# Gaeric/bevy-hikari

Measured on AMD Instinct MI355X. Metric: Mrays/sec + ms/frame @1080p 1spp; cornell & city scenes, 1/2/4/8 GPU, higher is better.
Workload: dtype f32

## Files before the change

### bevy-hikari_amd/csrc/hk_kernels.hip

```cpp
#include <stdlib.h>
#include <mutex>
#include <type_traits>

#include "hk_device.h"
#include "hk_launch.h"

namespace hk {

#ifdef HK_LANE_STATS
__device__ unsigned long long hk_lane_stats_dev[2 * LANE_SLOTS];
#endif
bool lane_stats_take(unsigned long long out[2 * LANE_SLOTS], hipStream_t st)
{
#ifdef HK_LANE_STATS
    unsigned long long zero[2 * LANE_SLOTS] = {};
    if (hipStreamSynchronize(st) != hipSuccess) return false;
    if (hipMemcpyFromSymbol(out, HIP_SYMBOL(hk_lane_stats_dev), sizeof(zero)) != hipSuccess) return false;
    return hipMemcpyToSymbol(HIP_SYMBOL(hk_lane_stats_dev), zero, sizeof(zero)) == hipSuccess;
#else
    (void)st;
    for (int k = 0; k < 2 * LANE_SLOTS; ++k) out[k] = 0;
    return false;
#endif
}
// ... 2320 lines not shown
    const bool window = A.F.upscale_ratio == 1.0f && A.F.s[0] == A.F.S[0] && A.F.s[1] == A.F.S[1];
    auto launch = [&](auto EL, auto VIEW) {
        if (window) hipLaunchKernelGGL((k_spatial<EL, VIEW>), g, dim3(256), 0, st, A, C);
        else hipLaunchKernelGGL((k_spatial_nowin<EL, VIEW>), g, dim3(256), 0, st, A, C);
    };
    if (emissive_lit) launch(std::true_type{}, std::false_type{});
    else dispatch([&](auto VIEW) { launch(std::false_type{}, VIEW); }, C.view != nullptr);
}
void launch_demod(const FrameArgs& A, const DenoiseArgs& D, hipStream_t st)
{
    dim3 g = tiles(A.F, A.F.s[0], A.F.s_rows);
    dispatch([&](auto C3) { hipLaunchKernelGGL((k_demod3<C3 ? 3 : 2>), g, dim3(256), 0, st, A, D); }, D.channels == 3);
}
template <int C, int LEVEL>
static void launch_level(const FrameArgs& A, const DenoiseArgs& D, hipStream_t st)
{
    const dim3 g = level_tiles<LEVEL>(launch_cols(A.F, A.F.s[0]), launch_rows(A.F, A.F.s_rows));
    hipLaunchKernelGGL((k_denoise3<C, LEVEL>), g, dim3(256), 0, st, A, D);
}
void launch_denoise(const FrameArgs& A, const DenoiseArgs& D, int level, hipStream_t st)
{
    dispatch(
        [&](auto C3) {
            constexpr int C = C3 ? 3 : 2;
            switch (level) {
            case 0: launch_level<C, 0>(A, D, st); break;
            case 1: launch_level<C, 1>(A, D, st); break;
            case 2: launch_level<C, 2>(A, D, st); break;
            default: launch_level<C, 3>(A, D, st); break;
            }
        },
        D.channels == 3);
}
void launch_tone(const FrameArgs& A, const ToneArgs& T, hipStream_t st)
{
    const Frame& F = A.F;
    const int32_t ly0 = F.win_rows > 0 ? F.win_row0 : 0, rows = launch_rows(F, F.s_rows);
    const int32_t x0 = F.win_cols > 0 ? F.win_col0 : 0, cols = (int32_t)launch_cols(F, F.s[0]);
    if (F.s[0] % (uint32_t)TONE_RUN == 0u && x0 % TONE_RUN == 0 && cols % TONE_RUN == 0 && rows > 0 && cols > 0) {
        const uint32_t runs = (uint32_t)cols / (uint32_t)TONE_RUN, n = runs * (uint32_t)rows;
        hipLaunchKernelGGL(k_tone_run, dim3((n + 255u) / 256u), dim3(256), 0, st, A, T, ly0, x0, runs, n);
    } else {
        hipLaunchKernelGGL(k_tone, tiles(A.F, A.F.s[0], A.F.s_rows), dim3(256), 0, st, A, T);
    }
}
__global__ __launch_bounds__(256) void k_accumulate(const uint2* tone, float4* acc, uint32_t n, int reset)
{
    uint32_t i = blockIdx.x * 256u + threadIdx.x;
    if (i >= n) return;
    f4 t = load_rgba16f(tone, (int32_t)i);
    float4 a = reset ? make_float4(0, 0, 0, 0) : acc[i];
    acc[i] = make_float4(a.x + t.x, a.y + t.y, a.z + t.z, a.w + t.w);
}
__global__ __launch_bounds__(256) void k_resolve(const float4* acc, uint32_t n, float count, uint2* out)
{
    uint32_t i = blockIdx.x * 256u + threadIdx.x;
    if (i >= n) return;
    float4 a = acc[i];
    store_rgba16f(out, (int32_t)i, mk4(a.x / count, a.y / count, a.z / count, a.w / count));
}
void launch_accumulate(const uint2* tone, float4* acc, uint32_t n, int reset, hipStream_t st)
{
    if (n) hipLaunchKernelGGL(k_accumulate, dim3((n + 255u) / 256u), dim3(256), 0, st, tone, acc, n, reset);
}
void launch_resolve(const float4* acc, uint32_t n, float count, uint2* out, hipStream_t st)
{
    if (n) hipLaunchKernelGGL(k_resolve, dim3((n + 255u) / 256u), dim3(256), 0, st, acc, n, count, out);
}

__global__ __launch_bounds__(256) void k_fill_blas_leaves(hk_node* nodes, uint32_t n, const uint32_t* prim_offset,
                                                          const hk_primitive* prims)
{
// ... 276 lines not shown
```

### bevy-hikari_amd/csrc/hk_launch.h

```cpp
#pragma once

#include <hip/hip_runtime.h>
#include <stdint.h>

#include "hk_device.h"
#include "../../include/hk_post.h"
#include "../../include/hk_fsr.h"
#include "../../include/hk_overlay.h"

namespace hk {

struct LaunchOpts {
    int lds_scene = 1;
    int gbuffer_stack_full = 0;
    int gbuffer_deep = 0;
    double gbuffer_lds_max_px = 6e5;
    double direct_w4_min_px = 4e5;
    int fused_w4 = 1;
    int persistent_indirect = 0;
    int compact_emitter = 0;
    int compact_shadow = 0;
};

struct FrameArgs {
// ... 184 lines not shown
    hk_pp_out out;
    hk_fsr_easu_con easu;
    float rcas;
};
void launch_fsr_easu(const FsrArgs& A, bool tiled, hipStream_t st);
void launch_fsr_rcas(const FsrArgs& A, hipStream_t st);

struct OverlayArgs {
    hk_pp_tex in, albedo;
    uint8_t* data;
    uint32_t pitch;
    hk_overlay_view view;
    uint32_t col0, cols;
};
void launch_overlay(const OverlayArgs& A, bool run, hipStream_t st);

bool lane_stats_take(unsigned long long out[2 * LANE_SLOTS], hipStream_t st);
void launch_gbuffer(const FrameArgs& A, const ViewArgs& V, uint2* albedo, uint32_t stack_need, hipStream_t st);
void launch_direct_fused(const FrameArgs& A, const ChannelArgs& C0, const ChannelArgs& C1, hipStream_t st,
                         const TileKeep& keep = TILE_KEEP_ALL);
void launch_albedo(const FrameArgs& A, uint2* albedo, hipStream_t st);
void launch_direct(const FrameArgs& A, const ChannelArgs& C, bool emissive_lit, hipStream_t st,
                   const TileKeep& keep = TILE_KEEP_ALL);
void launch_indirect(const FrameArgs& A, const ChannelArgs& C, bool multi, hipStream_t st, const TileKeep& keep = TILE_KEEP_ALL);
uint32_t indirect_stash_bytes();
void launch_indirect_wavefront(const FrameArgs& A, const ChannelArgs& C, const WfArgs& W, hipStream_t st);
void launch_spatial(const FrameArgs& A, const ChannelArgs& C, bool emissive_lit, hipStream_t st);
bool light_lds_direct(const FrameArgs& A);
void launch_light_merged(const FrameArgs& A, const ChannelArgs& C0, const ChannelArgs& C1, const ChannelArgs& C2,
                         hipStream_t st, const TileKeep& keep_direct = TILE_KEEP_ALL,
                         const TileKeep& keep_indirect = TILE_KEEP_ALL);
void launch_demod(const FrameArgs& A, const DenoiseArgs& D, hipStream_t st);
void launch_denoise(const FrameArgs& A, const DenoiseArgs& D, int level, hipStream_t st);
void launch_tone(const FrameArgs& A, const ToneArgs& T, hipStream_t st);
void launch_collapse_leaves(hk_node* nodes, uint32_t n, const uint32_t* node_base, const uint32_t* node_count,
                            uint32_t* scratch, hipStream_t st);
void launch_fill_leaves(hk_node* blas, uint32_t n_blas, const uint32_t* prim_offset, const hk_primitive* prims,
                        hk_node* tlas, uint32_t n_tlas, const hk_instance* inst, uint32_t n_inst, hipStream_t st);
void launch_build_wide(const hk_node* flat, uint32_t n, const uint32_t* node_base, const uint32_t* node_count,
                       float4* wide, hipStream_t st);
void launch_accumulate(const uint2* tone, float4* acc, uint32_t n, int reset, hipStream_t st);
void launch_resolve(const float4* acc, uint32_t n, float count, uint2* out, hipStream_t st);
void launch_div_check(float d, float r, uint32_t lo, uint32_t hi, unsigned long long* bad, hipStream_t st);
void launch_rcp_check(uint32_t lo, uint32_t hi, unsigned long long* bad, hipStream_t st);
void launch_count_check(const uint32_t* values, uint32_t n, unsigned long long* sum, hipStream_t st);
void launch_f16(const float* in, uint32_t n, uint16_t* out, hipStream_t st);
bool launch_math(int fn, const uint32_t* a, const uint32_t* b, const float* rb, uint32_t n, uint32_t* out0,
                 uint32_t* out1, hipStream_t st);
void launch_texture_check(const Scene& sc, uint32_t id, const float* uv, uint32_t n, float* out, hipStream_t st);
void launch_trace(const Scene& sc, const float* rays, const float* max_d, const float* early_d, const uint32_t* excl,
                  uint32_t n, uint32_t* hits, unsigned long long* top, hipStream_t st);

}
```

### bevy-hikari_amd/csrc/hk_runtime.hip

```cpp
#include <hip/hip_runtime.h>

#include <algorithm>
#include <array>
#include <cmath>
#include <cstdio>
#include <cstring>
#include <map>
#include <set>
#include <string>
#include <vector>

#include "../../include/hikari_amd.h"
#include "../../include/hikari_scene.h"
#include "hk_launch.h"

using namespace hk;

namespace {
constexpr int32_t BAND_HALO = 40;
constexpr size_t COUNTER_SPAN = (size_t)COUNTER_SHARDS * COUNTER_STRIDE;
constexpr size_t COUNTER_BYTES = 3 * COUNTER_SPAN * sizeof(unsigned long long);
constexpr size_t PERSIST_BYTES = (size_t)PERSIST_KINDS * PERSIST_LINES * PERSIST_LINE * sizeof(unsigned long long);

struct TimedLaunch {
// ... 203 lines not shown
        return PxRect{std::min(x0, o.x0), std::min(y0, o.y0), std::max(x1, o.x1), std::max(y1, o.y1)};
    }
};
struct MaskHistory {
    static constexpr int BITS = 5;
    PxRect cover[BITS];
    bool known[BITS] = {};
    void reset()
    {
        for (bool& k : known) k = false;
    }
    bool launch(uint32_t need, const PxRect& now, PxRect& keep)
    {
        bool ok = true;
        keep = now;
        for (int b = 0; b < BITS; ++b) {
            if (!(need >> b & 1u)) continue;
            if (!known[b]) ok = false;
            else keep = keep.join(cover[b]);
        }
        for (int b = 0; b < BITS; ++b) {
            if (need >> b & 1u) {
                cover[b] = now;
                known[b] = true;
            } else if (b == 4) {
                known[b] = false;
            } else if (known[b]) {
                cover[b] = cover[b].join(now);
            }
        }
        return ok;
    }
};
}

struct hk_ctx {
    int device = 0;
    hipStream_t stream = nullptr;
    std::string error;
    double opt[OPT_COUNT];
    bool on(Opt o) const { return opt[o] != 0.0; }

    void* buf[9] = {};
    uint32_t count[9] = {};
    hk_node* walk_nodes[2] = {nullptr, nullptr};
    uint32_t* collapse_scratch = nullptr;
    float4* blas_wide = nullptr;
    float4* tlas_wide = nullptr;
    uint32_t gb_stack_need = 0;
    bool heavy = false;
    int dn_calls = 0;
    uint32_t gb_blas_depth = 0;
    void* dyn_scratch = nullptr;
    size_t dyn_bytes = 0;
    struct MeshSlice {
        hk_mesh_index index;
        uint32_t vertex_need;
        uint32_t depth;
        uint32_t used = 0;
    };
    std::vector<MeshSlice> meshes;
    size_t cap[9] = {};
    size_t collapse_cap = 0;
    std::vector<float> emissive;
    uint32_t* blas_aux = nullptr;
    size_t aux_stride = 0;
// ... 13 lines not shown
    float* tex_lut = nullptr;
    uint32_t n_textures = 0;

    uint32_t S[2] = {0, 0}, s[2] = {0, 0};
    float ratio = 1.0f;
    int32_t S_row0 = 0, S_rows = 0, s_row0 = 0, s_rows = 0;
    int32_t core_row0 = 0, core_rows = 0;
    int32_t halo = BAND_HALO;
    int32_t stripe_n = 0, stripe_k = 0;
    bool albedo_fresh = false;
    bool sized = false;

    GSlot g, g_prev;
    FrameSchedule sch;
    uint32_t head = 0;
    float* variance[3] = {}, *variance_alt[3] = {};
    uint2* render[3] = {}, *render_alt[3] = {};
    uint4* reservoirs[HK_RESERVOIR_BUFFERS] = {};
    uint32_t res_n = 0;
    uint8_t* bgmask[2] = {};
    bool bg_valid[2] = {false, false};
    int32_t win_out = -1, win_emi = -1, win_ind = -1;
    int32_t core_col0 = 0, core_cols = 0;
    int32_t bg_key[2][2] = {};
    uint8_t* gbmask = nullptr;
    uint4* sp_view = nullptr;
    bool gb_valid = false;
    int32_t gb_key[2] = {};
    double scene_box[6] = {};
    bool scene_box_valid = false;
    PxRect grect[2] = {PxRect::all(), PxRect::all()};
    MaskHistory gb_hist, bg_hist[2];
    uint32_t tiles_skipped[3] = {};
    uint4* dn_rgb[4] = {};
    uint2* dn_bi[4] = {};
    float* internal_variance[3] = {};
    float4* dn_nd = nullptr;
    float4* dn_center = nullptr;
    float* dn_den2 = nullptr;
    int last_denoised_channels = 3;
    uint2* denoised[3] = {};
    uint2* tone_buf[2] = {};
    uint2* upscale = nullptr;
    uint2* taa_buf[2] = {};
    uint32_t upscale_wh[2] = {0, 0}, taa_wh[2] = {0, 0};
    uint2* fsr_buf[2] = {};
    float fsr_sharpness = 0.0f;
    uint8_t* present_buf = nullptr;
    uint32_t present_wh[2] = {0, 0}, present_format = 0;
    float4* accum = nullptr;
    uint2* accum_out = nullptr;
    uint32_t accum_n = 0;
    unsigned long long* counters = nullptr;
    unsigned long long* persist = nullptr;
    bool wavefront = false;
    uint32_t* wf_queue1 = nullptr;
    uint32_t* wf_keys = nullptr;
    uint32_t* wf_queue2 = nullptr;
    uint4* wf_hit = nullptr;
    float* wf_hit_t = nullptr;
    uint32_t* wf_ctl = nullptr;
    uint32_t wf_seg_cap = 0;

    struct GbSig {
        float view[3 + 16 + 16 + 16 + 2];
        int32_t win[2];
// ... 105 lines not shown
    for (auto& r : c->reservoirs) add(r, 's', 4);
    for (auto& m : c->bgmask) add(m, 's', 1, false);
    add(c->gbmask, 'S', 1, false);
    add(c->sp_view, 's', VIEW_PLANES);
    for (int i = 0; i < 4; ++i) {
        add(c->dn_rgb[i], 's');
        add(c->dn_bi[i], 's');
    }
    add(c->dn_nd, 's');
    add(c->dn_center, 's');
    add(c->dn_den2, 's');
    for (auto& b : c->tone_buf) add(b, 's');
    add(c->upscale, 0);
    for (auto& b : c->taa_buf) add(b, 0);
    for (auto& b : c->fsr_buf) add(b, 0);
    add(c->present_buf, 0);
    add(c->accum, 0);
    add(c->accum_out, 0);
    add(c->wf_queue1, 0);
    add(c->wf_keys, 0);
    add(c->wf_queue2, 0);
    add(c->wf_hit, 0);
    add(c->wf_hit_t, 0);
    add(c->wf_ctl, 0);
    return t;
}

void free_targets(hk_ctx* c)
{
    for (const Target& t : targets(c)) release(*t.ptr);
    c->bg_valid[0] = c->bg_valid[1] = c->gb_valid = false;
    c->grect[0] = c->grect[1] = PxRect::all();
    c->tiles_skipped[0] = c->tiles_skipped[1] = c->tiles_skipped[2] = 0;
    c->upscale_wh[0] = c->upscale_wh[1] = c->taa_wh[0] = c->taa_wh[1] = 0;
    c->present_wh[0] = c->present_wh[1] = 0;
    c->accum_n = 0;
    c->sch.reset();
    c->sized = false;
}

int ensure_wavefront(hk_ctx* c)
{
    if (c->wf_ctl) return HK_OK;
    const size_t n = (size_t)c->s[0] * (size_t)c->s_rows;
    const size_t tiles = (size_t)((c->s[0] + 15u) / 16u) * (size_t)(((uint32_t)c->s_rows + 15u) / 16u);
    c->wf_seg_cap = (uint32_t)(256u * ((tiles + WF_SEGS - 1u) / WF_SEGS));
    HK_HIP(c, hipMalloc(&c->wf_queue1, (size_t)WF_SEGS * c->wf_seg_cap * 4));
    HK_HIP(c, hipMalloc(&c->wf_keys, (size_t)WF_SEGS * c->wf_seg_cap * 4));
    HK_HIP(c, hipMalloc(&c->wf_queue2, n * 4));
    HK_HIP(c, hipMalloc(&c->wf_hit, n * sizeof(uint4)));
    HK_HIP(c, hipMalloc(&c->wf_hit_t, n * 4));
    HK_HIP(c, hipMalloc(&c->wf_ctl, (size_t)wf_ctl_words(WF_MAX_BINS) * 4));
    return HK_OK;
}

hipEvent_t take_event(hk_ctx* c)
{
    if (!c->event_pool.empty()) {
        hipEvent_t e = c->event_pool.back();
        c->event_pool.pop_back();
        return e;
    }
    hipEvent_t e = nullptr;
    (void)hipEventCreate(&e);
    return e;
}
// ... 272 lines not shown
    if (!G.grows) return HK_OK;
    commit_growth(c, G);
    if (!G.fill) return HK_OK;
    const size_t w = c->s[0];
    for (int b = 0; b < HK_RESERVOIR_BUFFERS; ++b)
        for (int side = 0; side < 2; ++side) {
            const int32_t r0 = G.rows[b][side][0], r1 = G.rows[b][side][1];
            if (r1 <= r0) continue;
            for (uint32_t plane = 0; plane < 4; ++plane)
                HK_HIP(c, hipMemsetAsync(c->reservoirs[b] + (size_t)plane * c->res_n + (size_t)r0 * w, 0,
                                         (size_t)(r1 - r0) * w * sizeof(uint4), s));
        }
    c->bg_valid[0] = c->bg_valid[1] = false;
    return HK_OK;
}


uint64_t gbuffer_primary_rays(const FrameArgs& A)
{
    const Frame& F = A.F;
    const int32_t w0 = F.win_rows > 0 ? F.win_row0 : 0, w1 = w0 + launch_rows(F, F.S_rows);
    if (F.stripe_n >= 2) return (uint64_t)F.S[0] * (uint64_t)(w1 - w0);
    const int32_t lo = std::max(F.S_row0 + w0, F.count_Sy0), hi = std::min(F.S_row0 + w1, F.count_Sy1);
    const int32_t c0 = F.win_cols > 0 ? F.win_col0 : 0, c1 = c0 + (int32_t)launch_cols(F, F.S[0]);
    const int32_t x0 = std::max(c0, F.count_x0), x1 = std::min(c1, F.count_x1);
    return hi > lo && x1 > x0 ? (uint64_t)(x1 - x0) * (uint64_t)(hi - lo) : 0u;
}

TileKeep tile_keep(const FrameArgs& A, uint32_t width, int32_t row0, int32_t rows, const PxRect& keep, uint32_t* skipped)
{
    const Frame& F = A.F;
    *skipped = 0;
    if (F.stripe_n >= 2) return TILE_KEEP_ALL;
    const int64_t ox = F.win_cols > 0 ? F.win_col0 : 0, oy = (int64_t)row0 + (F.win_rows > 0 ? F.win_row0 : 0);
    const int64_t gx = (launch_cols(F, width) + 15u) / 16u, gy = ((uint32_t)launch_rows(F, rows) + 15u) / 16u;
    auto lo = [](int64_t p, int64_t o, int64_t g) { return std::clamp<int64_t>(p - o, 0, 16 * g) / 16; };
    auto hi = [](int64_t p, int64_t o, int64_t g) { return (std::clamp<int64_t>(p - o, 0, 16 * g) + 15) / 16; };
    TileKeep K{(uint32_t)lo(keep.x0, ox, gx), (uint32_t)lo(keep.y0, oy, gy), (uint32_t)hi(keep.x1, ox, gx),
               (uint32_t)hi(keep.y1, oy, gy)};
    if (keep.empty() || K.x1 <= K.x0 || K.y1 <= K.y0) K = TileKeep{0u, 0u, 0u, 0u};
    *skipped = (uint32_t)(gx * gy) - (K.x1 - K.x0) * (K.y1 - K.y0);
    return *skipped ? K : TILE_KEEP_ALL;
}
uint64_t gbuffer_skipped_rays(const FrameArgs& A, const TileKeep& K)
{
    const Frame& F = A.F;
    const uint64_t all = gbuffer_primary_rays(A);
    if (K.x1 <= K.x0 || K.y1 <= K.y0) return all;
    const int32_t w0 = F.win_rows > 0 ? F.win_row0 : 0, w1 = w0 + launch_rows(F, F.S_rows);
    const int32_t c0 = F.win_cols > 0 ? F.win_col0 : 0, c1 = c0 + (int32_t)launch_cols(F, F.S[0]);
    const int32_t ky0 = std::min<int64_t>(w0 + 16 * (int64_t)K.y0, w1), ky1 = std::min<int64_t>(w0 + 16 * (int64_t)K.y1, w1);
    const int32_t kx0 = std::min<int64_t>(c0 + 16 * (int64_t)K.x0, c1), kx1 = std::min<int64_t>(c0 + 16 * (int64_t)K.x1, c1);
    const int32_t lo = std::max(F.S_row0 + ky0, F.count_Sy0), hi = std::min(F.S_row0 + ky1, F.count_Sy1);
    const int32_t x0 = std::max(kx0, F.count_x0), x1 = std::min(kx1, F.count_x1);
    const uint64_t kept = hi > lo && x1 > x0 ? (uint64_t)(x1 - x0) * (uint64_t)(hi - lo) : 0u;
    return all - kept;
}

int check_ready(hk_ctx* c, bool need_scene)
{
    if (!c) return HK_ERR_INVALID;
    if (!c->sized) return fail(c, HK_ERR_STATE, "hk_resize has not been called");
    if (need_scene && !c->has_scene) return fail(c, HK_ERR_STATE, "no scene uploaded (hk_scene_upload)");
    if (need_scene && !c->has_noise) return fail(c, HK_ERR_STATE, "no blue noise uploaded (hk_set_noise)");
    return HK_OK;
}

}

extern "C" {

int hk_abi_version(void) { return HK_ABI_VERSION; }

// ... 1411 lines not shown
{
    if (!c || !capacity) return HK_ERR_INVALID;
    if (!c->has_scene) return HK_ERR_STATE;
    for (int i = 0; i < 9; ++i) capacity[i] = (uint32_t)c->cap[i];
    return HK_OK;
}

int hk_scene_shared_transform(const hk_ctx* c, int32_t* shared)
{
    if (!c || !shared) return HK_ERR_INVALID;
    if (!c->has_scene) return HK_ERR_STATE;
    *shared = c->shared_transform ? 1 : 0;
    return HK_OK;
}

int hk_tile_skip_info(const hk_ctx* c, uint32_t skipped[3], int32_t bound[4], int32_t* bounded)
{
    if (!c) return HK_ERR_INVALID;
    if (!c->sized) return HK_ERR_STATE;
    if (skipped)
        for (int k = 0; k < 3; ++k) skipped[k] = c->tiles_skipped[k];
    const PxRect& r = c->grect[c->sch.gslot];
    const bool none = r.x1 == INT32_MAX;
    if (bound) {
        bound[0] = none ? 0 : r.x0;
        bound[1] = none ? 0 : r.y0;
        bound[2] = none ? (int32_t)c->S[0] : r.x1;
        bound[3] = none ? (int32_t)c->S[1] : r.y1;
    }
    if (bounded) *bounded = none ? 0 : 1;
    return HK_OK;
}

int hk_instance_set_counts(const hk_scene_desc* d, const hk_instance_desc* set, uint32_t count,
                           const hk_material* materials, uint32_t counts[9])
{
    if (!d || !set || !counts || !scene_desc_ok(d)) return HK_ERR_INVALID;
    const uint32_t before[9] = {d->vertices.count,  d->primitives.count,     d->asset_nodes.count,
                                d->alias_table.count, d->instances.count,    d->instance_nodes.count,
                                d->materials.count, d->emissive_nodes.count, d->emissives.count};
    std::vector<hk_ctx::MeshSlice> known;
    std::set<std::array<uint32_t, 4>> seen;
    const hk_instance* inst = (const hk_instance*)d->instances.data;
    for (uint32_t k = 0; k < d->instances.count; ++k) {
        const hk_mesh_index& m = inst[k].mesh;
        if ((size_t)m.node[0] + m.node[1] > d->asset_nodes.count) return HK_ERR_INVALID;
        if (seen.insert({m.vertex, m.primitive, m.node[0], m.node[1]}).second) known.push_back(host_mesh_slice(d, m));
    }
    std::vector<float> emissive(4 * (size_t)d->materials.count);
    const hk_material* mats = materials ? materials : (const hk_material*)d->materials.data;
    for (uint32_t k = 0; k < d->materials.count; ++k) std::memcpy(&emissive[4 * (size_t)k], mats[k].emissive, 16);
    SetChange change;
    std::string why;
    const int rc = plan_instance_set(before, known, emissive.data(), set, count, SliceReader{d, nullptr}, &change, &why);
    if (rc != HK_OK) return rc;
    std::memcpy(counts, change.counts, sizeof(change.counts));
    return HK_OK;
}

int hk_read_scene_array(hk_ctx* c, int array, void* dst, size_t bytes)
{
    if (!c || !dst || array < 0 || array > 8) return HK_ERR_INVALID;
    if (!c->has_scene) return fail(c, HK_ERR_STATE, "no scene uploaded (hk_scene_upload)");
    const size_t elem[9] = {sizeof(hk_vertex), sizeof(hk_primitive), sizeof(hk_node), sizeof(hk_alias_entry),
                            sizeof(hk_instance), sizeof(hk_node), sizeof(hk_material), sizeof(hk_node),
                            sizeof(hk_emissive)};
// ... 600 lines not shown
    D.den2 = c->dn_den2;
    c->last_denoised_channels = channels;
    const FrameArgs AD = pass_window(c, A, DENOISE_OUT_REACH - 1);
    timed(c, "demodulation", st, [&] { launch_demod(AD, D, st); });
    static constexpr int32_t LEVEL_REACH[4] = {7, 3, 1, 0};
    for (int level = 0; level < 4; ++level) {
        const FrameArgs AL = pass_window(c, A, LEVEL_REACH[level]);
        timed(c, "denoise", st, [&] { launch_denoise(AL, D, level, st); });
    }
    if (async) HK_TRY(c->sch.tail_end());
    HK_HIP(c, hipGetLastError());
    return HK_OK;
}

int hk_tone_sum(hk_ctx* c, const hk_settings* settings, void* stream)
{
    int rc = check_ready(c, false);
    if (rc) return rc;
    if (!settings) return fail(c, HK_ERR_INVALID, "null settings");
    (void)hipSetDevice(c->device);
    const bool async = c->sch.rf_swapped;
    hipStream_t st = async ? c->sch.dn_stream : pick_frame(c, stream);
    if (async) HK_TRY(c->sch.tail_begin());
    else HK_TRY(c->sch.gb_join(st));
    hk_frame_inputs dummy;
    std::memset(&dummy, 0, sizeof(dummy));
    const FrameArgs A = pass_window(c, frame_args(c, settings, &dummy), 0);
    ToneArgs T;
    T.direct = settings->denoise ? c->denoised[0] : c->render[0];
    T.emissive = settings->denoise ? c->denoised[1] : c->render[1];
    T.indirect = settings->indirect_bounces == 0u ? nullptr : (settings->denoise ? c->denoised[2] : c->render[2]);
    T.output = c->tone_buf[c->head];
    HK_TRY(c->sch.ext_wait(st, T.output));
    timed(c, "tone_mapping", st, [&] { launch_tone(A, T, st); });
    if (async) HK_TRY(c->sch.tail_end());
    HK_HIP(c, hipGetLastError());
    return HK_OK;
}

int hk_post_process(hk_ctx* c, const hk_settings* st, const hk_frame_inputs* in, void* stream)
{
    int rc = check_ready(c, false);
    if (rc) return rc;
    if (!st || !in) return fail(c, HK_ERR_INVALID, "null settings or frame inputs");
    if (c->S_rows != (int32_t)c->S[1]) return fail(c, HK_ERR_STATE, "hk_post_process (SMAA TU4x, TAA, FSR1) needs a whole-frame context");
    (void)hipSetDevice(c->device);
    hipStream_t s = pick(c, stream);
    HK_TRY(c->sch.gb_join(s));
    c->head = in->frame_number & 1u;
    const uint32_t head = c->head;
    HK_TRY(c->sch.ext_wait(s, c->upscale));
    HK_TRY(c->sch.ext_wait(s, c->taa_buf[head]));
    for (auto& b : c->fsr_buf) HK_TRY(c->sch.ext_wait(s, b));
    float scale = 1.0f / c->ratio;
    const bool smaa = st->upscale == 0u, fsr = st->upscale == 1u, taa = st->taa == 0u;
    PostArgs P;
    P.frame.number = in->frame_number;
    for (int k = 0; k < 4; ++k) P.frame.clear_color[k] = st->clear_color[k];
    P.frame.upscale_ratio = c->ratio;
    auto tex = [](const void* d, uint32_t w, uint32_t h, uint32_t f16, uint32_t comps) {
        hk_pp_tex t;
        t.data = d, t.w = w, t.h = h, t.f16 = f16, t.comps = comps;
        return t;
    };
    const uint32_t S0 = c->S[0], S1 = c->S[1];
    P.in.position = tex(c->g.position, S0, S1, 0, 4);
    P.in.previous_position = tex(c->g_prev.position, S0, S1, 0, 4);
// ... 719 lines not shown
```

### bevy-hikari_amd/csrc/hk_scene.cpp

```cpp
#include "../../include/hikari_scene.h"

#include <algorithm>
#include <cmath>
#include <cstring>
#include <limits>
#include <string>
#include <vector>

namespace {

struct V3 {
    float x, y, z;
};
static inline V3 v3(float x, float y, float z) { return V3{x, y, z}; }
static inline V3 operator+(V3 a, V3 b) { return v3(a.x + b.x, a.y + b.y, a.z + b.z); }
static inline V3 operator-(V3 a, V3 b) { return v3(a.x - b.x, a.y - b.y, a.z - b.z); }
static inline V3 operator*(V3 a, float s) { return v3(a.x * s, a.y * s, a.z * s); }
static inline V3 vmin(V3 a, V3 b) { return v3(std::fmin(a.x, b.x), std::fmin(a.y, b.y), std::fmin(a.z, b.z)); }
static inline V3 vmax(V3 a, V3 b) { return v3(std::fmax(a.x, b.x), std::fmax(a.y, b.y), std::fmax(a.z, b.z)); }
static inline float dot(V3 a, V3 b) { return a.x * b.x + a.y * b.y + a.z * b.z; }
static inline V3 cross(V3 a, V3 b)
{
    return v3(a.y * b.z - b.y * a.z, a.z * b.x - b.z * a.x, a.x * b.y - b.x * a.y);
}
// ... 532 lines not shown
        const double eye[3] = {view->world_position[0], view->world_position[1], view->world_position[2]};
        double c[4];
        clip(eye, c);
        for (int r : {0, 1, 3}) {
            const double scale = std::fabs((double)m[r]) * std::fabs(eye[0]) + std::fabs((double)m[4 + r]) * std::fabs(eye[1]) +
                                 std::fabs((double)m[8 + r]) * std::fabs(eye[2]) + std::fabs((double)m[12 + r]);
            if (!(std::fabs(c[r]) <= 1e-4 * scale + 1e-12)) return 0;
        }
        near_w = std::fmax(0.0, (double)view->projection[14]);
    }
    double lo[2] = {INFINITY, INFINITY}, hi[2] = {-INFINITY, -INFINITY};
    for (int corner = 0; corner < 8; ++corner) {
        const double p[3] = {aabb[(corner & 1) ? 3 : 0], aabb[(corner & 2) ? 4 : 1], aabb[(corner & 4) ? 5 : 2]};
        double c[4];
        clip(p, c);
        if (!std::isfinite(c[0]) || !std::isfinite(c[1]) || !std::isfinite(c[2]) || !std::isfinite(c[3])) return 0;
        if (ortho ? !(c[3] > 0.0 && c[2] < c[3]) : !(c[3] > near_w && c[3] > 1e-9)) return 0;
        const double px = (c[0] / c[3] + 1.0) * 0.5 * (double)width, py = (1.0 - c[1] / c[3]) * 0.5 * (double)height;
        lo[0] = std::fmin(lo[0], px);
        hi[0] = std::fmax(hi[0], px);
        lo[1] = std::fmin(lo[1], py);
        hi[1] = std::fmax(hi[1], py);
    }
    const double size[2] = {(double)width, (double)height};
    for (int a = 0; a < 2; ++a) {
        const double p0 = std::floor(lo[a] - 0.5) - (double)guard, p1 = std::ceil(hi[a] + 0.5) + 1.0 + (double)guard;
        rect[a] = (int32_t)std::fmin(std::fmax(p0, 0.0), size[a]);
        rect[2 + a] = (int32_t)std::fmin(std::fmax(p1, 0.0), size[a]);
    }
    if (rect[2] <= rect[0] || rect[3] <= rect[1]) rect[0] = rect[1] = rect[2] = rect[3] = 0;
    return 1;
}

}
```

### bevy-hikari_amd/hikari_amd/_abi.py

```python
from __future__ import annotations

import ctypes as C
import os
from pathlib import Path

HERE = Path(__file__).resolve().parent
LIB_PATH = Path(os.environ["HK_LIB"]) if os.environ.get("HK_LIB") else HERE / "libhikari_amd.so"

HK_OK = 0
HK_ERR_INVALID = -1
HK_ERR_HIP = -2
HK_ERR_STATE = -3
HK_ERR_NO_DEVICE = -4

RESERVOIR_BUFFERS = 10

MATH_FN_NAMES = (
    "exp2", "exp", "exp_weight", "log2", "pow", "pow2", "pow5", "pow16", "sincos",
    "unorm16", "snorm8", "unpack_unorm16_fast", "unpack_snorm8_fast", "unorm8_fast", "random_float",
    "fract", "minf", "maxf", "saturate", "signf",
    "div", "sqrt", "rcp_exact", "rcp_fast", "div_by", "f2u32", "f2i32", "unpack_f16",
)
MATH_FN = {name: i for i, name in enumerate(MATH_FN_NAMES)}
MATH_FN_TWO_OPERANDS = ("pow", "unpack_snorm8_fast", "minf", "maxf", "div", "div_by")
# ... 202 lines not shown
        "hk_resolve_accumulation": (i32, [vp, vp]),
        "hk_output_info": (i32, [vp, i32, C.POINTER(u32), C.POINTER(u32), C.POINTER(u32)]),
        "hk_get_output": (i32, [vp, i32, vp, C.c_size_t, i32, vp]),
        "hk_output_device_ptr": (vp, [vp, i32]),
        "hk_sync": (i32, [vp, vp]),
        "hk_set_wavefront": (i32, [vp, i32]),
        "hk_lane_stats": (i32, [vp, C.POINTER(C.c_char_p), C.POINTER(C.c_uint64), C.POINTER(C.c_uint64), i32]),
        "hk_dump_reservoirs": (i32, [vp, i32, vp, C.c_size_t, vp]),
        "hk_load_reservoirs": (i32, [vp, i32, vp, C.c_size_t, vp]),
        "hk_reset_counters": (i32, [vp, vp]),
        "hk_read_counters": (i32, [vp, C.POINTER(hk_counters), vp]),
        "hk_enable_kernel_timing": (i32, [vp, i32]),
        "hk_kernel_timing": (i32, [vp, C.POINTER(C.c_char_p), C.POINTER(C.c_float), i32]),
        "hk_set_kernel_timing_interval": (i32, [vp, u32]),
        "hk_trace": (i32, [vp, vp, vp, vp, vp, u32, vp, i32, vp]),
        "hk_selftest_f16": (i32, [vp, vp, u32, vp]),
        "hk_selftest_div": (i32, [vp, C.c_float, u32, u32, C.POINTER(C.c_uint64)]),
        "hk_selftest_rcp": (i32, [vp, u32, u32, C.POINTER(C.c_uint64)]),
        "hk_selftest_count": (i32, [vp, vp, u32, C.POINTER(C.c_uint64)]),
        "hk_selftest_texture": (i32, [vp, u32, vp, u32, vp]),
        "hk_selftest_math": (i32, [vp, i32, vp, vp, u32, vp, vp]),
        "hks_create": (vp, []),
        "hks_destroy": (None, [vp]),
        "hks_last_error": (C.c_char_p, [vp]),
        "hks_add_mesh": (i32, [vp, vp, vp, vp, u32, vp, u32, i32]),
        "hks_add_material": (i32, [vp, vp]),
        "hks_add_instance": (i32, [vp, u32, u32, vp]),
        "hks_build": (i32, [vp, i32]),
        "hks_get_desc": (i32, [vp, C.POINTER(hk_scene_desc)]),
        "hks_shared_transform": (i32, [vp, u32]),
        "hks_instance_bounds": (i32, [vp, vp, u32, C.POINTER(C.c_double)]),
        "hks_screen_bounds": (i32, [C.POINTER(C.c_double), C.POINTER(hk_view), u32, u32, u32, C.POINTER(i32)]),
        "hk_tile_skip_info": (i32, [vp, C.POINTER(u32), C.POINTER(i32), C.POINTER(i32)]),
    }
    for name, (res, args) in sig.items():
        f = getattr(L, name)
        f.restype = res
        f.argtypes = args
    _lib = L
    return L


EXPORTED_SYMBOLS = [
    "hk_abi_version", "hk_create", "hk_destroy", "hk_last_error", "hk_settings_default", "hk_set_option",
    "hk_get_option", "hk_option_name", "hk_scene_upload", "hk_scene_stage_bytes", "hk_scene_indirect_lds",
    "hk_scene_gbuffer_stack",
    "hk_set_noise", "hk_texture_upload", "hk_resize", "hk_resize_striped", "hk_set_band_halo", "hk_band_info", "hk_band_window_grow", "hk_reservoir_rows", "hk_resize_tile", "hk_tile_info", "hk_copy_output_rect", "hk_copy_output_rows", "hk_render_gbuffer", "hk_set_gbuffer_plane", "hk_render_frame",
    "hk_denoise", "hk_tone_sum", "hk_update_instances", "hk_update_meshes", "hk_set_instances", "hk_scene_counts", "hk_instance_set_counts", "hk_read_scene_array", "hk_post_process", "hk_set_fsr1_sharpness", "hk_present", "hk_present_info", "hk_get_present", "hk_accumulate", "hk_resolve_accumulation", "hk_output_info", "hk_get_output", "hk_output_device_ptr", "hk_sync", "hk_set_wavefront", "hk_lane_stats", "hk_dump_reservoirs",
    "hk_load_reservoirs", "hk_reset_counters", "hk_read_counters", "hk_enable_kernel_timing", "hk_kernel_timing", "hk_set_kernel_timing_interval",
    "hk_trace", "hk_selftest_f16", "hk_selftest_div", "hk_selftest_rcp", "hk_selftest_count", "hk_selftest_texture", "hk_selftest_math", "hks_create", "hks_destroy", "hks_last_error", "hks_add_mesh", "hks_add_material",
    "hks_add_instance", "hks_build", "hks_get_desc", "hk_scene_shared_transform", "hks_shared_transform",
    "hks_instance_bounds", "hks_screen_bounds", "hk_tile_skip_info",
    "hk_add_meshes", "hk_add_meshes_counts", "hk_add_meshes_counts_error", "hk_scene_capacity",
    "hk_set_meshes", "hk_set_meshes_counts", "hk_set_meshes_counts_error",
]


def gpu_visible() -> bool:
    return bool(os.environ.get("HIP_VISIBLE_DEVICES", "x")) and Path("/dev/kfd").exists()
```

### bevy-hikari_amd/hikari_amd/plugin.py

```python
from __future__ import annotations

import ctypes as C
from typing import Optional

import numpy as np

from . import _abi
from .scene import Mesh, Scene, load_noise, texture_array
from .settings import HikariSettings, HikariUniversalSettings, PresentFormat

RESERVOIR_DTYPE = np.dtype([("radiance", "<u4", 2), ("random", "<u4", 2), ("visible_position", "<f4", 4),
                            ("sample_position", "<f4", 4), ("visible_normal", "<u4"), ("sample_normal", "<u4"),
                            ("reservoir", "<u4", 2)])
assert RESERVOIR_DTYPE.itemsize == 64


def _stream(stream):
    if stream is None or isinstance(stream, (int, C.c_void_p)):
        return stream
    raise TypeError(f"stream must be None or an integer hipStream_t handle, not {type(stream).__name__}")


def _check(ctx, rc: int, what: str) -> None:
    if rc != 0:
# ... 303 lines not shown
    def set_meshes(self, scene: Scene, entries, previous=None, materials: bool = False, models=None, local_aabbs=None,
                   stream=None) -> list:
        m = np.ascontiguousarray(scene.instance_models() if models is None else models, np.float32).reshape(-1, 16)
        a = np.ascontiguousarray(scene.instance_local_aabbs() if local_aabbs is None else local_aabbs,
                                 np.float32).reshape(-1, 6)
        if len(m) != len(a) or len(m) != len(scene.instances):
            raise ValueError("models and local_aabbs need one record per instance")
        if len(entries) != len(scene.meshes):
            raise ValueError("entries needs one item per mesh of the scene")
        arr, keep = _mesh_entries(entries)
        slices = (_abi.hk_mesh_index * max(1, len(entries)))()
        mats = material_records(scene) if materials else None
        _check(self.ctx, self._L.hk_set_meshes(self.ctx, arr, len(entries), slices, instance_descs(scene, previous),
                                               m.ctypes.data, a.ctypes.data, len(m), mats, _stream(stream)),
               "hk_set_meshes")
        return [(s.vertex, s.primitive, s.node[0], s.node[1]) for s in slices[:len(entries)]]

    def scene_capacity(self) -> list:
        out = (C.c_uint32 * 9)()
        _check(self.ctx, self._L.hk_scene_capacity(self.ctx, out), "hk_scene_capacity")
        return list(out)

    def scene_shared_transform(self) -> bool:
        out = C.c_int32()
        _check(self.ctx, self._L.hk_scene_shared_transform(self.ctx, C.byref(out)), "hk_scene_shared_transform")
        return bool(out.value)

    def tile_skip_info(self) -> dict:
        skipped, bound, bounded = (C.c_uint32 * 3)(), (C.c_int32 * 4)(), C.c_int32()
        _check(self.ctx, self._L.hk_tile_skip_info(self.ctx, skipped, bound, C.byref(bounded)), "hk_tile_skip_info")
        return {"gbuffer": skipped[0], "direct": skipped[1], "indirect": skipped[2],
                "bound": tuple(bound) if bounded.value else None}

    def scene_array(self, array: int, dtype, count: int) -> np.ndarray:
        out = np.empty(count, dtype)
        _check(self.ctx, self._L.hk_read_scene_array(self.ctx, array, out.ctypes.data, out.nbytes),
               "hk_read_scene_array")
        return out

    def post_process(self, settings: _abi.hk_settings, inputs: _abi.hk_frame_inputs, stream=None) -> None:
        _check(self.ctx, self._L.hk_post_process(self.ctx, C.byref(settings), C.byref(inputs), _stream(stream)),
               "hk_post_process")

    def set_fsr1_sharpness(self, sharpness: float) -> None:
        _check(self.ctx, self._L.hk_set_fsr1_sharpness(self.ctx, float(sharpness)), "hk_set_fsr1_sharpness")

    def present(self, settings, width: int, height: int, format="rgba8_srgb", viewport=None, input: int = -1,
                dst_ptr: Optional[int] = None, pitch: int = 0, stream=None):
        t = _abi.hk_present_target()
        t.data, t.width, t.height, t.pitch = dst_ptr, int(width), int(height), int(pitch)
        t.format = int(PresentFormat.of(format))
        t.vp_x, t.vp_y, t.vp_w, t.vp_h = (0, 0, 0, 0) if viewport is None else [int(v) for v in viewport]
        t.input = int(input)
        _check(self.ctx, self._L.hk_present(self.ctx, None if settings is None else C.byref(settings), C.byref(t),
                                            _stream(stream)), "hk_present")
        return self.get_present(stream) if dst_ptr is None else None

    def present_info(self):
        v = [C.c_uint32() for _ in range(4)]
        _check(self.ctx, self._L.hk_present_info(self.ctx, *[C.byref(x) for x in v]), "hk_present_info")
        return v[0].value, v[1].value, v[2].value, PresentFormat(v[3].value)

    def get_present(self, stream=None) -> np.ndarray:
        w, h, b, _ = self.present_info()
        out = np.empty((h, w, 4), np.uint8 if b == 4 else np.uint16)
        _check(self.ctx, self._L.hk_get_present(self.ctx, out.ctypes.data, out.nbytes, 1, _stream(stream)),
# ... 188 lines not shown
```

### include/hikari_amd.h

```cpp
#ifndef HIKARI_AMD_H
#define HIKARI_AMD_H

#include <stddef.h>
#include <stdint.h>
#include "hk_types.h"
#include "hk_texture.h"

#ifdef __cplusplus
extern "C" {
#endif

#define HK_ABI_VERSION 3

enum {
    HK_OK = 0,
    HK_ERR_INVALID = -1,
    HK_ERR_HIP = -2,
    HK_ERR_STATE = -3,
    HK_ERR_NO_DEVICE = -4,
};

typedef struct hk_ctx hk_ctx;

typedef struct hk_array {
// ... 131 lines not shown
} hk_instance_desc;
int hk_set_instances(hk_ctx* ctx, const hk_instance_desc* set, const float* models, const float* local_aabbs,
                     uint32_t count, const hk_material* materials, void* stream);
int hk_scene_counts(const hk_ctx* ctx, uint32_t counts[9]);

typedef struct hk_mesh_desc {
    const float* positions;
    const float* normals;
    const float* uvs;
    uint32_t vertex_count;
    const uint32_t* indices;
    uint32_t index_count;
    uint32_t topology;
} hk_mesh_desc;
int hk_add_meshes(hk_ctx* ctx, const hk_mesh_desc* meshes, uint32_t mesh_count, hk_mesh_index* slices, void* stream);
int hk_add_meshes_counts(const uint32_t before[9], const hk_mesh_desc* meshes, uint32_t mesh_count,
                         hk_mesh_index* slices, uint32_t after[9]);
const char* hk_add_meshes_counts_error(void);

typedef struct hk_mesh_entry {
    const hk_mesh_desc* source;
    hk_mesh_index keep;
    uint32_t vertex_count;
} hk_mesh_entry;
int hk_set_meshes(hk_ctx* ctx, const hk_mesh_entry* list, uint32_t mesh_count, hk_mesh_index* slices,
                  const hk_instance_desc* set, const float* models, const float* local_aabbs, uint32_t count,
                  const hk_material* materials, void* stream);
int hk_set_meshes_counts(const uint32_t before[9], const hk_mesh_entry* list, uint32_t mesh_count,
                         hk_mesh_index* slices, uint32_t after[9]);
const char* hk_set_meshes_counts_error(void);
int hk_scene_capacity(const hk_ctx* ctx, uint32_t capacity[9]);
int hk_scene_shared_transform(const hk_ctx* ctx, int32_t* shared);
int hk_tile_skip_info(const hk_ctx* ctx, uint32_t skipped[3], int32_t bound[4], int32_t* bounded);
int hk_instance_set_counts(const hk_scene_desc* uploaded, const hk_instance_desc* set, uint32_t count,
                           const hk_material* materials, uint32_t counts[9]);
int hk_scene_stage_bytes(const hk_scene_desc* scene, int plan, uint32_t* bytes, uint32_t* limit);
int hk_scene_indirect_lds(const hk_scene_desc* scene, uint32_t* stash, uint32_t* total, uint32_t* limit);
int hk_scene_gbuffer_stack(const hk_scene_desc* scene, uint32_t* need, uint32_t* lds_levels);
int hk_read_scene_array(hk_ctx* ctx, int array, void* dst, size_t bytes);

int hk_post_process(hk_ctx* ctx, const hk_settings* settings, const hk_frame_inputs* inputs, void* stream);
int hk_set_fsr1_sharpness(hk_ctx* ctx, float sharpness);

enum { HK_PRESENT_RGBA8_SRGB = 0, HK_PRESENT_BGRA8_SRGB = 1, HK_PRESENT_RGBA16F = 2 };
typedef struct hk_present_target {
    void*    data;
    uint32_t width, height;
    uint32_t pitch;
    uint32_t format;
    uint32_t vp_x, vp_y, vp_w, vp_h;
    int32_t  input;
} hk_present_target;
int hk_present(hk_ctx* ctx, const hk_settings* settings, const hk_present_target* target, void* stream);
int hk_present_info(const hk_ctx* ctx, uint32_t* width, uint32_t* height, uint32_t* bytes_per_texel, uint32_t* format);
int hk_get_present(hk_ctx* ctx, void* dst, size_t bytes, int to_host, void* stream);

int hk_accumulate(hk_ctx* ctx, int reset, void* stream);
int hk_resolve_accumulation(hk_ctx* ctx, void* stream);

typedef struct hk_texture {
    uint32_t width, height;
    uint32_t format;
    uint32_t address_u, address_v;
    uint32_t filter;
    const uint8_t* rgba8;
} hk_texture;
// ... 89 lines not shown
```

### include/hikari_scene.h

```cpp
#ifndef HIKARI_SCENE_H
#define HIKARI_SCENE_H

#include <stdint.h>
#include "hikari_amd.h"

#ifdef __cplusplus
extern "C" {
#endif

typedef struct hks_scene hks_scene;

enum { HKS_TRIANGLE_LIST = 0, HKS_TRIANGLE_STRIP = 1 };

hks_scene* hks_create(void);
void hks_destroy(hks_scene* scene);
const char* hks_last_error(const hks_scene* scene);

int hks_add_mesh(hks_scene* scene, const float* positions, const float* normals, const float* uvs,
                 uint32_t vertex_count, const uint32_t* indices, uint32_t index_count, int topology);
int hks_add_material(hks_scene* scene, const hk_material* material);
int hks_add_instance(hks_scene* scene, uint32_t mesh, uint32_t material, const float* model);

int hks_build(hks_scene* scene, int buckets);
int hks_get_desc(const hks_scene* scene, hk_scene_desc* out);

int hks_shared_transform(const float* matrices, uint32_t n);

int hks_instance_bounds(const float* models, const float* local_aabbs, uint32_t n, double aabb[6]);
int hks_screen_bounds(const double aabb[6], const hk_view* view, uint32_t width, uint32_t height, uint32_t guard,
                      int32_t rect[4]);

#ifdef __cplusplus
}
#endif

#endif
```

Measured before the change: 12070.

## Restrict tone mapping launch to rectangle covering non-background pixels

Tracks per-buffer history of which screen rectangle held non-background content and, when the background is known to be unchanged (same clear color and window, no denoise), launches the tone-mapping kernel only over the union of the current and previous covered rectangles. Pixels outside that rectangle keep their prior tone output in the ring buffer. The tile-keep computation is factored into a shared helper, and introspection APIs are added. It adds host-side bookkeeping and relies on the ring buffer still holding valid background pixels from earlier frames.

```diff
diff --git a/bevy-hikari_amd/csrc/hk_kernels.hip b/bevy-hikari_amd/csrc/hk_kernels.hip
--- a/bevy-hikari_amd/csrc/hk_kernels.hip
+++ b/bevy-hikari_amd/csrc/hk_kernels.hip
@@ -2376,12 +2376,25 @@
         },
         D.channels == 3);
 }
-void launch_tone(const FrameArgs& A, const ToneArgs& T, hipStream_t st)
+uint32_t tone_run_px(const FrameArgs& A)
 {
     const Frame& F = A.F;
-    const int32_t ly0 = F.win_rows > 0 ? F.win_row0 : 0, rows = launch_rows(F, F.s_rows);
+    const int32_t rows = launch_rows(F, F.s_rows);
     const int32_t x0 = F.win_cols > 0 ? F.win_col0 : 0, cols = (int32_t)launch_cols(F, F.s[0]);
-    if (F.s[0] % (uint32_t)TONE_RUN == 0u && x0 % TONE_RUN == 0 && cols % TONE_RUN == 0 && rows > 0 && cols > 0) {
+    return F.s[0] % (uint32_t)TONE_RUN == 0u && x0 % TONE_RUN == 0 && cols % TONE_RUN == 0 && rows > 0 && cols > 0 ? (uint32_t)TONE_RUN : 0u;
+}
+void launch_tone(const FrameArgs& A, const ToneArgs& T, hipStream_t st, const int32_t* rect)
+{
+    const Frame& F = A.F;
+    int32_t ly0 = F.win_rows > 0 ? F.win_row0 : 0, rows = launch_rows(F, F.s_rows);
+    int32_t x0 = F.win_cols > 0 ? F.win_col0 : 0, cols = (int32_t)launch_cols(F, F.s[0]);
+    if (tone_run_px(A)) {
+        if (rect) {
+            const int32_t rx0 = std::max(rect[0], x0) / TONE_RUN * TONE_RUN, rx1 = std::min(rect[2], x0 + cols);
+            const int32_t ry0 = std::max(rect[1], ly0), ry1 = std::min(rect[3], ly0 + rows);
+            if (rx1 <= rx0 || ry1 <= ry0) return;
+            x0 = rx0, cols = (rx1 - rx0 + TONE_RUN - 1) / TONE_RUN * TONE_RUN, ly0 = ry0, rows = ry1 - ry0;
+        }
         const uint32_t runs = (uint32_t)cols / (uint32_t)TONE_RUN, n = runs * (uint32_t)rows;
         hipLaunchKernelGGL(k_tone_run, dim3((n + 255u) / 256u), dim3(256), 0, st, A, T, ly0, x0, runs, n);
     } else {
diff --git a/bevy-hikari_amd/csrc/hk_launch.h b/bevy-hikari_amd/csrc/hk_launch.h
--- a/bevy-hikari_amd/csrc/hk_launch.h
+++ b/bevy-hikari_amd/csrc/hk_launch.h
@@ -240,7 +240,8 @@
                          const TileKeep& keep_indirect = TILE_KEEP_ALL);
 void launch_demod(const FrameArgs& A, const DenoiseArgs& D, hipStream_t st);
 void launch_denoise(const FrameArgs& A, const DenoiseArgs& D, int level, hipStream_t st);
-void launch_tone(const FrameArgs& A, const ToneArgs& T, hipStream_t st);
+void launch_tone(const FrameArgs& A, const ToneArgs& T, hipStream_t st, const int32_t* rect = nullptr);
+uint32_t tone_run_px(const FrameArgs& A);
 void launch_collapse_leaves(hk_node* nodes, uint32_t n, const uint32_t* node_base, const uint32_t* node_count,
                             uint32_t* scratch, hipStream_t st);
 void launch_fill_leaves(hk_node* blas, uint32_t n_blas, const uint32_t* prim_offset, const hk_primitive* prims,
diff --git a/bevy-hikari_amd/csrc/hk_runtime.hip b/bevy-hikari_amd/csrc/hk_runtime.hip
--- a/bevy-hikari_amd/csrc/hk_runtime.hip
+++ b/bevy-hikari_amd/csrc/hk_runtime.hip
@@ -259,6 +259,17 @@
         return ok;
     }
 };
+struct ToneHistory {
+    bool known = false;
+    PxRect cover;
+    float clear[4] = {};
+    int32_t key[4] = {};
+    void reset() { known = false; }
+    bool holds(const float* clear_color, const int32_t* window) const
+    {
+        return known && std::memcmp(clear, clear_color, sizeof(clear)) == 0 && std::memcmp(key, window, sizeof(key)) == 0;
+    }
+};
 }
 
 struct hk_ctx {
@@ -338,6 +349,9 @@
     PxRect grect[2] = {PxRect::all(), PxRect::all()};
     MaskHistory gb_hist, bg_hist[2];
     uint32_t tiles_skipped[3] = {};
+    ToneHistory tone_hist[2];
+    uint64_t tone_skipped = 0;
+    int32_t tone_rect[4] = {};
     uint4* dn_rgb[4] = {};
     uint2* dn_bi[4] = {};
     float* internal_variance[3] = {};
@@ -509,6 +523,10 @@
     c->bg_valid[0] = c->bg_valid[1] = c->gb_valid = false;
     c->grect[0] = c->grect[1] = PxRect::all();
     c->tiles_skipped[0] = c->tiles_skipped[1] = c->tiles_skipped[2] = 0;
+    c->tone_hist[0].reset();
+    c->tone_hist[1].reset();
+    c->tone_skipped = 0;
+    c->tone_rect[0] = c->tone_rect[1] = c->tone_rect[2] = c->tone_rect[3] = 0;
     c->upscale_wh[0] = c->upscale_wh[1] = c->taa_wh[0] = c->taa_wh[1] = 0;
     c->present_wh[0] = c->present_wh[1] = 0;
     c->accum_n = 0;
@@ -847,13 +865,13 @@
     const Frame& F = A.F;
     *skipped = 0;
     if (F.stripe_n >= 2) return TILE_KEEP_ALL;
-    const int64_t ox = F.win_cols > 0 ? F.win_col0 : 0, oy = (int64_t)row0 + (F.win_rows > 0 ? F.win_row0 : 0);
+    const int32_t ox = F.win_cols > 0 ? F.win_col0 : 0, oy = F.win_rows > 0 ? F.win_row0 : 0;
+    const int32_t window[4] = {ox, oy, ox + (int32_t)launch_cols(F, width), oy + launch_rows(F, rows)};
     const int64_t gx = (launch_cols(F, width) + 15u) / 16u, gy = ((uint32_t)launch_rows(F, rows) + 15u) / 16u;
-    auto lo = [](int64_t p, int64_t o, int64_t g) { return std::clamp<int64_t>(p - o, 0, 16 * g) / 16; };
-    auto hi = [](int64_t p, int64_t o, int64_t g) { return (std::clamp<int64_t>(p - o, 0, 16 * g) + 15) / 16; };
-    TileKeep K{(uint32_t)lo(keep.x0, ox, gx), (uint32_t)lo(keep.y0, oy, gy), (uint32_t)hi(keep.x1, ox, gx),
-               (uint32_t)hi(keep.y1, oy, gy)};
-    if (keep.empty() || K.x1 <= K.x0 || K.y1 <= K.y0) K = TileKeep{0u, 0u, 0u, 0u};
+    const int32_t kr[4] = {keep.x0, keep.y0, keep.x1, keep.y1};
+    uint32_t t[4];
+    (void)hks_keep_tiles(kr, window, row0, 16u, t);
+    const TileKeep K{t[0], t[1], t[2], t[3]};
     *skipped = (uint32_t)(gx * gy) - (K.x1 - K.x0) * (K.y1 - K.y0);
     return *skipped ? K : TILE_KEEP_ALL;
 }
@@ -2331,6 +2349,16 @@
     return HK_OK;
 }
 
+int hk_tone_skip_info(const hk_ctx* c, uint64_t* skipped_pixels, int32_t rect[4])
+{
+    if (!c) return HK_ERR_INVALID;
+    if (!c->sized) return HK_ERR_STATE;
+    if (skipped_pixels) *skipped_pixels = c->tone_skipped;
+    if (rect)
+        for (int k = 0; k < 4; ++k) rect[k] = c->tone_rect[k];
+    return HK_OK;
+}
+
 int hk_instance_set_counts(const hk_scene_desc* d, const hk_instance_desc* set, uint32_t count,
                            const hk_material* materials, uint32_t counts[9])
 {
@@ -2997,7 +3025,37 @@
     T.indirect = settings->indirect_bounces == 0u ? nullptr : (settings->denoise ? c->denoised[2] : c->render[2]);
     T.output = c->tone_buf[c->head];
     HK_TRY(c->sch.ext_wait(st, T.output));
-    timed(c, "tone_mapping", st, [&] { launch_tone(A, T, st); });
+    const int32_t ly0 = A.F.win_rows > 0 ? A.F.win_row0 : 0, x0 = A.F.win_cols > 0 ? A.F.win_col0 : 0;
+    const int32_t window[4] = {x0, ly0, x0 + (int32_t)launch_cols(A.F, A.F.s[0]), ly0 + launch_rows(A.F, A.F.s_rows)};
+    const int32_t key[4] = {window[1], window[3] - window[1], window[0], window[2] - window[0]};
+    const uint32_t run = tone_run_px(A);
+    PxRect in = PxRect::all();
+    bool in_known = run != 0u && !settings->denoise && !bg_elision_off(c) && c->on(OPT_BG_TILE_SKIP) && c->stripe_n < 2;
+    for (int k = 0; in_known && k < (T.indirect ? 2 : 1); ++k) {
+        const int bit = 2 + (int)c->sch.rslot;
+        in_known = c->bg_valid[k] && c->bg_hist[k].known[bit];
+        if (in_known) in = k == 0 ? c->bg_hist[k].cover[bit] : in.join(c->bg_hist[k].cover[bit]);
+    }
+    ToneHistory& H = c->tone_hist[c->head];
+    const int64_t all_px = (int64_t)(window[2] - window[0]) * (int64_t)(window[3] - window[1]);
+    int32_t rect[4] = {window[0], window[1], window[2], window[3]};
+    bool any = true;
+    if (in_known && H.holds(settings->clear_color, key)) {
+        const PxRect keep = in.join(H.cover);
+        const int32_t kr[4] = {keep.x0, keep.y0, keep.x1, keep.y1};
+        any = hks_tone_rect(kr, window, c->s_row0, run, rect) != 0;
+    }
+    if (in_known) {
+        H.known = true;
+        H.cover = in;
+        std::memcpy(H.clear, settings->clear_color, sizeof(H.clear));
+        std::memcpy(H.key, key, sizeof(H.key));
+    } else {
+        H.reset();
+    }
+    c->tone_skipped = (uint64_t)(all_px - (any ? (int64_t)(rect[2] - rect[0]) * (int64_t)(rect[3] - rect[1]) : 0));
+    for (int k = 0; k < 4; ++k) c->tone_rect[k] = any ? rect[k] + ((k & 1) ? c->s_row0 : 0) : 0;
+    if (any) timed(c, "tone_mapping", st, [&] { launch_tone(A, T, st, c->tone_skipped ? rect : nullptr); });
     if (async) HK_TRY(c->sch.tail_end());
     HK_HIP(c, hipGetLastError());
     return HK_OK;
diff --git a/bevy-hikari_amd/csrc/hk_scene.cpp b/bevy-hikari_amd/csrc/hk_scene.cpp
--- a/bevy-hikari_amd/csrc/hk_scene.cpp
+++ b/bevy-hikari_amd/csrc/hk_scene.cpp
@@ -588,4 +588,38 @@
     return 1;
 }
 
-}
+int hks_keep_tiles(const int32_t keep[4], const int32_t window[4], int32_t row0, uint32_t tile, uint32_t tiles[4])
+{
+    if (!keep || !window || !tiles || tile == 0) return 0;
+    tiles[0] = tiles[1] = tiles[2] = tiles[3] = 0;
+    if (window[2] <= window[0] || window[3] <= window[1]) return 0;
+    if (keep[2] <= keep[0] || keep[3] <= keep[1]) return 0;
+    const int64_t t = (int64_t)tile, ox = window[0], oy = (int64_t)row0 + window[1];
+    const int64_t gx = ((int64_t)window[2] - window[0] + t - 1) / t, gy = ((int64_t)window[3] - window[1] + t - 1) / t;
+    auto lo = [t](int64_t p, int64_t o, int64_t g) { return std::clamp<int64_t>(p - o, 0, t * g) / t; };
+    auto hi = [t](int64_t p, int64_t o, int64_t g) { return (std::clamp<int64_t>(p - o, 0, t * g) + t - 1) / t; };
+    const int64_t x0 = lo(keep[0], ox, gx), y0 = lo(keep[1], oy, gy), x1 = hi(keep[2], ox, gx), y1 = hi(keep[3], oy, gy);
+    if (x1 <= x0 || y1 <= y0) return 0;
+    tiles[0] = (uint32_t)x0, tiles[1] = (uint32_t)y0, tiles[2] = (uint32_t)x1, tiles[3] = (uint32_t)y1;
+    return 1;
+}
+
+int hks_tone_rect(const int32_t keep[4], const int32_t window[4], int32_t row0, uint32_t run, int32_t launch[4])
+{
+    if (!keep || !window || !launch || run == 0) return 0;
+    launch[0] = launch[1] = launch[2] = launch[3] = 0;
+    const int64_t r = (int64_t)run;
+    if (window[0] < 0 || window[1] < 0 || window[2] <= window[0] || window[3] <= window[1]) return 0;
+    if (window[0] % r != 0 || window[2] % r != 0) return 0;
+    if (keep[2] <= keep[0] || keep[3] <= keep[1]) return 0;
+    const int64_t x0 = std::max<int64_t>(keep[0], window[0]), x1 = std::min<int64_t>(keep[2], window[2]);
+    const int64_t y0 = std::max<int64_t>((int64_t)keep[1] - row0, window[1]), y1 = std::min<int64_t>((int64_t)keep[3] - row0, window[3]);
+    if (x1 <= x0 || y1 <= y0) return 0;
+    launch[0] = (int32_t)(x0 / r * r);
+    launch[1] = (int32_t)y0;
+    launch[2] = (int32_t)((x1 + r - 1) / r * r);
+    launch[3] = (int32_t)y1;
+    return 1;
+}
+
+}
diff --git a/bevy-hikari_amd/hikari_amd/_abi.py b/bevy-hikari_amd/hikari_amd/_abi.py
--- a/bevy-hikari_amd/hikari_amd/_abi.py
+++ b/bevy-hikari_amd/hikari_amd/_abi.py
@@ -258,6 +258,9 @@
         "hks_instance_bounds": (i32, [vp, vp, u32, C.POINTER(C.c_double)]),
         "hks_screen_bounds": (i32, [C.POINTER(C.c_double), C.POINTER(hk_view), u32, u32, u32, C.POINTER(i32)]),
         "hk_tile_skip_info": (i32, [vp, C.POINTER(u32), C.POINTER(i32), C.POINTER(i32)]),
+        "hk_tone_skip_info": (i32, [vp, C.POINTER(C.c_uint64), C.POINTER(i32)]),
+        "hks_tone_rect": (i32, [C.POINTER(i32), C.POINTER(i32), i32, u32, C.POINTER(i32)]),
+        "hks_keep_tiles": (i32, [C.POINTER(i32), C.POINTER(i32), i32, u32, C.POINTER(u32)]),
     }
     for name, (res, args) in sig.items():
         f = getattr(L, name)
@@ -276,7 +279,7 @@
     "hk_load_reservoirs", "hk_reset_counters", "hk_read_counters", "hk_enable_kernel_timing", "hk_kernel_timing", "hk_set_kernel_timing_interval",
     "hk_trace", "hk_selftest_f16", "hk_selftest_div", "hk_selftest_rcp", "hk_selftest_count", "hk_selftest_texture", "hk_selftest_math", "hks_create", "hks_destroy", "hks_last_error", "hks_add_mesh", "hks_add_material",
     "hks_add_instance", "hks_build", "hks_get_desc", "hk_scene_shared_transform", "hks_shared_transform",
-    "hks_instance_bounds", "hks_screen_bounds", "hk_tile_skip_info",
+    "hks_instance_bounds", "hks_screen_bounds", "hk_tile_skip_info", "hk_tone_skip_info", "hks_tone_rect", "hks_keep_tiles",
     "hk_add_meshes", "hk_add_meshes_counts", "hk_add_meshes_counts_error", "hk_scene_capacity",
     "hk_set_meshes", "hk_set_meshes_counts", "hk_set_meshes_counts_error",
 ]
diff --git a/bevy-hikari_amd/hikari_amd/plugin.py b/bevy-hikari_amd/hikari_amd/plugin.py
--- a/bevy-hikari_amd/hikari_amd/plugin.py
+++ b/bevy-hikari_amd/hikari_amd/plugin.py
@@ -359,6 +359,11 @@
         return {"gbuffer": skipped[0], "direct": skipped[1], "indirect": skipped[2],
                 "bound": tuple(bound) if bounded.value else None}
 
+    def tone_skip_info(self) -> dict:
+        skipped, rect = C.c_uint64(), (C.c_int32 * 4)()
+        _check(self.ctx, self._L.hk_tone_skip_info(self.ctx, C.byref(skipped), rect), "hk_tone_skip_info")
+        return {"skipped": int(skipped.value), "rect": tuple(rect) if any(rect) else None}
+
     def scene_array(self, array: int, dtype, count: int) -> np.ndarray:
         out = np.empty(count, dtype)
         _check(self.ctx, self._L.hk_read_scene_array(self.ctx, array, out.ctypes.data, out.nbytes),
diff --git a/include/hikari_amd.h b/include/hikari_amd.h
--- a/include/hikari_amd.h
+++ b/include/hikari_amd.h
@@ -187,6 +187,7 @@
 int hk_scene_capacity(const hk_ctx* ctx, uint32_t capacity[9]);
 int hk_scene_shared_transform(const hk_ctx* ctx, int32_t* shared);
 int hk_tile_skip_info(const hk_ctx* ctx, uint32_t skipped[3], int32_t bound[4], int32_t* bounded);
+int hk_tone_skip_info(const hk_ctx* ctx, uint64_t* skipped_pixels, int32_t rect[4]);
 int hk_instance_set_counts(const hk_scene_desc* uploaded, const hk_instance_desc* set, uint32_t count,
                            const hk_material* materials, uint32_t counts[9]);
 int hk_scene_stage_bytes(const hk_scene_desc* scene, int plan, uint32_t* bytes, uint32_t* limit);
diff --git a/include/hikari_scene.h b/include/hikari_scene.h
--- a/include/hikari_scene.h
+++ b/include/hikari_scene.h
@@ -29,6 +29,8 @@
 int hks_instance_bounds(const float* models, const float* local_aabbs, uint32_t n, double aabb[6]);
 int hks_screen_bounds(const double aabb[6], const hk_view* view, uint32_t width, uint32_t height, uint32_t guard,
                       int32_t rect[4]);
+int hks_tone_rect(const int32_t keep[4], const int32_t window[4], int32_t row0, uint32_t run, int32_t launch[4]);
+int hks_keep_tiles(const int32_t keep[4], const int32_t window[4], int32_t row0, uint32_t tile, uint32_t tiles[4]);
 
 #ifdef __cplusplus
 }
```

After: 12300, median of 6. 1.02x the previous value.
